# DavidHuji/CapDec

Measured on AMD Instinct MI355X. Metric: captions/sec (whole node), COCO-val 5k, prefix_len=10 beam=5, 1/2/4/8 GPUs, higher is better.
Workload: dtype f32 (operands split into 2 fp16 planes, 3 fp16 MFMAs per product, fp32 accumulate); 1 GPU; COCO-val-5k-shaped: 5000 x 512-d synthetic CLIP embeddings in total (sharded over the ranks) -> normalise -> TransformerMapper(8 layers) -> GPT-2 small KV-cached beam-5 decode, prefix_len 10, entry_length 67, hot-init seeded weights (never emit the stop id: all 67 steps run); captions_per_gpu=5000, beam=5, parallelism=caption-shard dp1

## Files before the change

capdec_amd/csrc/attention.hip:

```cpp
#include <cstdlib>

#include "bf16x3.h"
#include "common.h"

namespace capdec {

constexpr int ATT_CTX_MAX = 1024;
#define ATT_BIG_LDS(K, bytes)                                                                                   \
    if ((bytes) > 64 * 1024)                                                                                    \
    CAPDEC_HIP(hipFuncSetAttribute((const void *)(K), hipFuncAttributeMaxDynamicSharedMemorySize, (int)(bytes)))
constexpr int ATT_MFMA_MIN_P = 24;
constexpr int ATT_MFMA_MAX_P = 128;

__device__ __forceinline__ float dot4(const float4 &a, const float4 &b) {
    return (a.x * b.x + a.y * b.y) + (a.z * b.z + a.w * b.w);
}
__device__ __forceinline__ float group16_sum(float v) { return row16_sum(v); }
__device__ __forceinline__ float groups4_sum(float v) {
    v += __shfl_xor(v, 16, 64);
    v += __shfl_xor(v, 32, 64);
    return v;
}

template <typename KV> struct KvIo;
// ... 467 lines not shown
#pragma unroll
    for (int t = 0; t < NT; ++t) {
        if (t < nt) {
#pragma unroll
            for (int s2 = 0; s2 < 2; ++s2) {
                f16x8 ph, pl;
#pragma unroll
                for (int e = 0; e < 8; ++e) {
                    const float p = sc[t][8 * s2 + e];
                    if constexpr (SPLIT) {
                        const _Float16 hh = p < 0x1p-14f ? (_Float16)0.f : (_Float16)p;
                        ph[e] = hh;
                        pl[e] = (_Float16)((p - (float)hh) * H2_LO_SCALE);
                    } else
                        ph[e] = (_Float16)p;
                }
#pragma unroll
                for (int n = 0; n < 2; ++n) {
                    const _Float16 *vr = Vt + (size_t)(32 * n + l32) * VST + 32 * t + 16 * s2 + 8 * half;
                    const f16x8 vh = *reinterpret_cast<const f16x8 *>(vr);
                    if constexpr (SPLIT) {
                        const f16x8 vl = *reinterpret_cast<const f16x8 *>(vr + (size_t)64 * VST);
                        oc[n] = __builtin_amdgcn_mfma_f32_32x32x16_f16(pl, vh, oc[n], 0, 0, 0);
                        om[n] = __builtin_amdgcn_mfma_f32_32x32x16_f16(ph, vh, om[n], 0, 0, 0);
                        oc[n] = __builtin_amdgcn_mfma_f32_32x32x16_f16(ph, vl, oc[n], 0, 0, 0);
                    } else
                        om[n] = __builtin_amdgcn_mfma_f32_32x32x16_f16(ph, vh, om[n], 0, 0, 0);
                }
            }
        }
    }
    __syncthreads();
    float *ost = reinterpret_cast<float *>(am_smem) + (size_t)wave * 32 * AM_OST;
#pragma unroll
    for (int r = 0; r < 16; ++r) {
        const int row = (r & 3) + 8 * (r >> 2) + 4 * half;
        const float li = __shfl(linv, row, 64);
#pragma unroll
        for (int n = 0; n < 2; ++n) ost[row * AM_OST + 32 * n + l32] = (SPLIT ? om[n][r] + oc[n][r] * LO : om[n][r]) * li;
    }
    __builtin_amdgcn_fence(__ATOMIC_RELEASE, "wavefront");
    __builtin_amdgcn_wave_barrier();
    __builtin_amdgcn_fence(__ATOMIC_ACQUIRE, "wavefront");
    for (int q = lane; q < 32 * 16; q += 64) {
        const int row = q >> 4, c4 = q & 15, grow = wave * 32 + row;
        if (grow >= S) continue;
        const float4 o = *reinterpret_cast<const float4 *>(ost + row * AM_OST + c4 * 4);
        const int orow = cap * S + grow;
        if (packed_out) x3_store_quad(packed_out, d >> 4, orow, head * 4 + (c4 >> 2), c4 & 3, o, fmt);
        else reinterpret_cast<float4 *>(out + (size_t)orow * d + head * 64)[c4] = o;
    }
}

template <typename KV>
__global__ void kv_scatter_prefill_kernel(const float *__restrict__ qkv, KV *__restrict__ kc,
                                          KV *__restrict__ vc, int ncap, int P, int beam, int heads, int ctx,
                                          int d) {
    const int nv = d / 4;
    const int i = blockIdx.x * blockDim.x + threadIdx.x;
    if (i >= ncap * P * nv) return;
    const int c4 = i % nv, row = i / nv;
    const int cap = row / P, pos = row - cap * P;
    const int head = (c4 * 4) / 64, within = (c4 * 4) % 64;
    const size_t o = (((size_t)cap * beam * heads + head) * ctx + pos) * 64 + within;
    const float *r = qkv + (size_t)row * 3 * d;
    KvIo<KV>::st4(kc + o, reinterpret_cast<const float4 *>(r + d)[c4]);
    KvIo<KV>::st4(vc + o, reinterpret_cast<const float4 *>(r + 2 * d)[c4]);
}

int launch_kv_scatter_prefill(hipStream_t st, const float *qkv, const KvCache &c, int layer, int ncap, int P,
                              int beam) {
    const int d = c.heads * c.hd;
    const int tot = ncap * P * (d / 4);
    if (tot <= 0) return 0;
    if (c.bf16)
        hipLaunchKernelGGL(kv_scatter_prefill_kernel<__bf16>, dim3((tot + 255) / 256), dim3(256), 0, st, qkv,
                           c.kp<__bf16>(layer), c.vp<__bf16>(layer), ncap, P, beam, c.heads, c.ctx, d);
    else
        hipLaunchKernelGGL(kv_scatter_prefill_kernel<float>, dim3((tot + 255) / 256), dim3(256), 0, st, qkv,
                           c.kp<float>(layer), c.vp<float>(layer), ncap, P, beam, c.heads, c.ctx, d);
    CAPDEC_HIP(hipGetLastError());
    return 0;
}

int launch_attn_prefill(hipStream_t st, const float *qkv, const KvCache &c, int layer, int ncap, int P, int beam,
                        float *out, bool causal, void *packed_out, int fmt) {
    CAPDEC_CHECK(c.hd == 64, "attention: head_dim must be 64");
    CAPDEC_CHECK(P <= ATT_CTX_MAX && P <= c.ctx, "attention: prefix longer than the supported context");
    (void)layer; (void)beam;
    const bool tower = c.k == nullptr;
    const bool split = !((fmt == PK_F16X1 || fmt == PK_BF16X1) && tower);
    if (!c.bf16 && (P >= ATT_MFMA_MIN_P || tower) && P <= ATT_MFMA_MAX_P && ncap > 0) {
        const int nqt = (P + 31) / 32;
        const size_t lds = attn_mfma_lds_bytes(P, split ? 2 : 1);
#define LAUNCH_AM(CZ, NTV)                                                                                          \
    {                                                                                                               \
        if (lds > 64 * 1024)       \
            CAPDEC_HIP(hipFuncSetAttribute((const void *)attn_prefill_mfma_kernel<CZ, NTV, true>,                   \
                                           hipFuncAttributeMaxDynamicSharedMemorySize, (int)lds));                  \
        if (split)                                                                                                  \
            hipLaunchKernelGGL((attn_prefill_mfma_kernel<CZ, NTV, true>), dim3(ncap * c.heads), dim3(64 * nqt), lds, st, qkv, \
                               c.heads, P, c.heads * c.hd, out, (char *)packed_out, fmt);                            \
        else                                                                                                        \
            hipLaunchKernelGGL((attn_prefill_mfma_kernel<CZ, NTV, false>), dim3(ncap * c.heads), dim3(64 * nqt), lds, st, qkv, \
                               c.heads, P, c.heads * c.hd, out, (char *)packed_out, fmt);                            \
    }
#define LAUNCH_AM_NT(CZ)                                                                                            \
    switch (nqt) {                                                                                                  \
        case 1: LAUNCH_AM(CZ, 1) break;                                                                             \
        case 2: LAUNCH_AM(CZ, 2) break;                                                                             \
        case 3: LAUNCH_AM(CZ, 3) break;                                                                             \
        default: LAUNCH_AM(CZ, 4) break;                                                                            \
    }
        if (causal) { LAUNCH_AM_NT(true) } else { LAUNCH_AM_NT(false) }
#undef LAUNCH_AM_NT
#undef LAUNCH_AM
        CAPDEC_HIP(hipGetLastError());
        return 0;
    }
    constexpr int R = 8;
    const int total = ncap * c.heads * ((P + R - 1) / R);
    if (total <= 0) return 0;
    const size_t lds = (size_t)4 * R * P * sizeof(float);
    CAPDEC_CHECK(lds <= 160 * 1024, "attention: prefix too long for the score rows in LDS");
    ATT_BIG_LDS((attn_prefill_rows_kernel<R, __bf16>), lds);
    ATT_BIG_LDS((attn_prefill_rows_kernel<R, float>), lds);
    if (c.bf16)
        hipLaunchKernelGGL((attn_prefill_rows_kernel<R, __bf16>), dim3((total + 3) / 4), dim3(256), lds, st, qkv, total,
                           c.heads, P, c.heads * c.hd, causal ? 1 : 0, out, (char *)packed_out, fmt);
    else
        hipLaunchKernelGGL((attn_prefill_rows_kernel<R, float>), dim3((total + 3) / 4), dim3(256), lds, st, qkv, total,
                           c.heads, P, c.heads * c.hd, causal ? 1 : 0, out, (char *)packed_out, fmt);
    CAPDEC_HIP(hipGetLastError());
    return 0;
}

template <typename KV>
static int attn_decode_typed(hipStream_t st, const float *qkv, const KvCache &c, int layer, int rows, int beam, int L,
                             const uint8_t *anc, int anc_stride, float *out, void *packed_out, const int *cmap,
                             int fmt, bool cur_cached) {
    KV *kl = c.kp<KV>(layer), *vl = c.vp<KV>(layer);
    const int npre = anc == nullptr ? L : c.prefix_len;
    {
        const int ncap = rows / beam, total = ncap * c.heads;
        if (total <= 0) return 0;
        size_t lds = ((size_t)4 * beam * L * sizeof(int) + 1023) & ~(size_t)1023;
        CAPDEC_CHECK(lds + 32 * 1024 <= 160 * 1024, "attention: context too long for the slot table in LDS");
        dim3 grid((total + 3) / 4), block(256);
        const bool na4 = !c.fixed_variant && total <= 16384;
#define LAUNCH_BEAMS_V(B, OCC, NAV, CURV)                                                                       \
    ATT_BIG_LDS((attn_decode_beams_kernel<B, KV, OCC, NAV, CURV, false>), lds);                                    \
    hipLaunchKernelGGL((attn_decode_beams_kernel<B, KV, OCC, NAV, CURV, false>), grid, block, lds, st, qkv, kl, vl, total, \
                       c.heads, c.ctx, c.heads * c.hd, L, anc, anc_stride, out, (char *)packed_out, cmap, fmt, npre, 0)
#define LAUNCH_BEAMS_DMA(B, OCC)                                                                                \
    ATT_BIG_LDS((attn_decode_beams_kernel<B, float, OCC, 2, true, true>), lds + 4 * 2 * (2 * 2 * 1024));          \
    hipLaunchKernelGGL((attn_decode_beams_kernel<B, float, OCC, 2, true, true>), grid, block, lds + 4 * 2 * (2 * 2 * 1024), st, \
                       qkv, (float *)kl, (float *)vl, total, c.heads, c.ctx, c.heads * c.hd, L, anc, anc_stride, out,  \
                       (char *)packed_out, cmap, fmt, npre, (int)lds)
#define LAUNCH_BEAMS_NA(B, OCC, CURV)                                                                           \
    if constexpr (B <= 5) {                                                                                     \
        if (na4) { LAUNCH_BEAMS_V(B, OCC, 4, CURV); } else { LAUNCH_BEAMS_V(B, OCC, 2, CURV); }                 \
    } else { LAUNCH_BEAMS_V(B, OCC, 2, CURV); }
#define LAUNCH_BEAMS(B, OCC)                                                                                    \
    if constexpr (B == 1 || B == 5) {                                                                           \
        if (!cur_cached) { LAUNCH_BEAMS_NA(B, OCC, false) }                                                     \
        else if constexpr (sizeof(KV) == 4) { LAUNCH_BEAMS_DMA(B, OCC); }                                       \
        else { LAUNCH_BEAMS_NA(B, OCC, true) }                                                                  \
    } else { LAUNCH_BEAMS_NA(B, OCC, false) }
        switch (beam) {
            case 1: LAUNCH_BEAMS(1, 4); break;
            case 2: LAUNCH_BEAMS(2, 4); break;
// ... 25 lines not shown
}

__global__ __launch_bounds__(256) void attn_mapper_kernel(const float *__restrict__ q, int ldq,
                                                          const float *__restrict__ k, const float *__restrict__ v,
                                                          int ldkv, float *__restrict__ out, int seq, int heads,
                                                          int hd, float scale) {
    extern __shared__ __attribute__((aligned(16))) float sm[];
    const int ld = hd + 1;
    float *Ks = sm;
    float *Vs = Ks + seq * ld;
    float *qb = Vs + seq * ld;
    float *pb = qb + 4 * hd;
    const int cap = blockIdx.x / heads, head = blockIdx.x - cap * heads;
    const int d = heads * hd;
    const int lane = threadIdx.x & 63, wave = threadIdx.x >> 6;
    for (int i = threadIdx.x; i < seq * hd; i += 256) {
        const int j = i / hd, c = i - j * hd;
        const size_t o = ((size_t)cap * seq + j) * ldkv + head * hd + c;
        Ks[j * ld + c] = k[o];
        Vs[j * ld + c] = v[o];
    }
    __syncthreads();
    for (int i = wave; i < seq; i += 4) {
        const float *qr = q + ((size_t)cap * seq + i) * ldq + head * hd;
        for (int c = lane; c < hd; c += 64) qb[wave * hd + c] = qr[c];
        __builtin_amdgcn_wave_barrier();
        float mx = -INFINITY;
        for (int j = lane; j < seq; j += 64) {
            float s = 0.f;
            for (int c = 0; c < hd; ++c) s += qb[wave * hd + c] * Ks[j * ld + c];
            s *= scale;
            pb[wave * seq + j] = s;
            mx = fmaxf(mx, s);
        }
        mx = wave_max(mx);
        float sum = 0.f;
        for (int j = lane; j < seq; j += 64) {
            const float e = expf(pb[wave * seq + j] - mx);
            pb[wave * seq + j] = e;
            sum += e;
        }
        sum = wave_sum(sum);
        __builtin_amdgcn_wave_barrier();
        const float inv = 1.0f / sum;
        for (int c = lane; c < hd; c += 64) {
            float a = 0.f;
            for (int j = 0; j < seq; ++j) a += pb[wave * seq + j] * Vs[j * ld + c];
            out[((size_t)cap * seq + i) * d + head * hd + c] = a * inv;
        }
        __builtin_amdgcn_wave_barrier();
    }
}

int launch_attn_mapper(hipStream_t st, const float *q, int ldq, const float *k, const float *v, int ldkv, float *out,
                       int n, int seq, int heads, int hd) {
    if (n <= 0) return 0;
    const size_t lds = ((size_t)2 * seq * (hd + 1) + 4 * hd + 4 * seq) * sizeof(float);
    CAPDEC_CHECK(lds <= 160 * 1024, "mapper attention: sequence too long for LDS");
    if (lds > 64 * 1024)
        CAPDEC_HIP(hipFuncSetAttribute((const void *)attn_mapper_kernel, hipFuncAttributeMaxDynamicSharedMemorySize,
                                       (int)lds));
    hipLaunchKernelGGL(attn_mapper_kernel, dim3(n * heads), dim3(256), lds, st, q, ldq, k, v, ldkv, out, seq, heads, hd,
                       (float)pow((double)hd, -0.5));
    CAPDEC_HIP(hipGetLastError());
    return 0;
}

__global__ __launch_bounds__(256) void attn_cross_kernel(const float *__restrict__ q, int ldq, size_t q_cap,
                                                         const float *__restrict__ k, const float *__restrict__ v,
                                                         int ldkv, float *__restrict__ out, int total, int nq, int nkv,
                                                         int heads, int hd, float scale, int group, int tj, int vec) {
    extern __shared__ __attribute__((aligned(16))) float sm[];
    const int ld = hd + 1;
    const int tpu = 256 / group, wpu = tpu >> 6;
    const int ul = threadIdx.x / tpu, tu = threadIdx.x - ul * tpu;
    const int unit = blockIdx.x * group + ul;
    const bool live = unit < total;
    float *Ks = sm + (size_t)ul * (2 * nkv * ld + nq * hd + wpu * nkv);
    float *Vs = Ks + nkv * ld;
    float *Qs = Vs + nkv * ld;
    const int cap = unit / heads, head = unit - cap * heads;
    const int lane = tu & 63, wave = tu >> 6;
    float *pw = Qs + nq * hd + wave * nkv;
    if (live) {
        const float *kb = k + (size_t)cap * nkv * ldkv + head * hd, *vb = v + (size_t)cap * nkv * ldkv + head * hd;
        const float *qb = q + (size_t)cap * q_cap + head * hd;
        if (vec) {
            const int hv = hd >> 2;
            for (int i = tu; i < nkv * hv; i += tpu) {
                const int j = i / hv, c = (i - j * hv) << 2;
                const float4 a = *reinterpret_cast<const float4 *>(kb + (size_t)j * ldkv + c);
                const float4 b = *reinterpret_cast<const float4 *>(vb + (size_t)j * ldkv + c);
                float *kd = Ks + j * ld + c, *vd = Vs + j * ld + c;
                kd[0] = a.x; kd[1] = a.y; kd[2] = a.z; kd[3] = a.w;
                vd[0] = b.x; vd[1] = b.y; vd[2] = b.z; vd[3] = b.w;
            }
            for (int i = tu; i < nq * hv; i += tpu) {
                const int r = i / hv, c = (i - r * hv) << 2;
                const float4 a = *reinterpret_cast<const float4 *>(qb + (size_t)r * ldq + c);
                float *qd = Qs + r * hd + c;
                qd[0] = a.x; qd[1] = a.y; qd[2] = a.z; qd[3] = a.w;
            }
        } else {
            for (int i = tu; i < nkv * hd; i += tpu) {
                const int j = i / hd, c = i - j * hd;
                Ks[j * ld + c] = kb[(size_t)j * ldkv + c];
                Vs[j * ld + c] = vb[(size_t)j * ldkv + c];
            }
            for (int i = tu; i < nq * hd; i += tpu) {
// ... 79 lines not shown
```

capdec_amd/csrc/common.h:

```cpp
#pragma once
#include <hip/hip_runtime.h>
#include <stdint.h>
#include <string>
#include <type_traits>
#include <vector>

#include "../../include/capdec.h"
#include "config.h"

namespace capdec {

void set_error(const std::string &msg);

#define CAPDEC_HIP(expr)                                                                         \
    do {                                                                                         \
        hipError_t _e = (expr);                                                                  \
        if (_e != hipSuccess) {                                                                  \
            ::capdec::set_error(std::string(#expr) + ": " + hipGetErrorString(_e) + " (" +       \
                                __FILE__ + ":" + std::to_string(__LINE__) + ")");               \
            return 1;                                                                            \
        }                                                                                        \
    } while (0)

#define CAPDEC_CHECK(cond, msg)                                                                  \
// ... 158 lines not shown
                     int ldy, int rows, int d);
int launch_l2norm_rows(hipStream_t st, const float *x, void *packed, float *y, int rows, int d, int fmt, int *row_bad,
                       int *any_bad);
int launch_embed_tokens(hipStream_t st, const int *tok, const float *wte, const float *wpe_row, float *h, int rows,
                        int d, const int *cmap = nullptr, int beam = 1);
int launch_embed_prefix(hipStream_t st, const float *prefix, const float *wpe, float *h, int n, int P, int pos0,
                        int d);
int launch_gather_rows(hipStream_t st, const float *table, const int *ids, float *out, int rows, int d);
int launch_normalize_prefix(hipStream_t st, const float *x, int n, int dim, int normalize, const float *offset,
                            float *out);
int launch_noise_inject(hipStream_t st, const float *x, int n, int dim, float variance, const float *offset,
                        int uniform, int dont_norm, uint64_t seed, const float *noise, const float *u, float *out);
int launch_tmapper_concat(hipStream_t st, const float *lin, const float *prefix_const, float *seq, int n,
                          int clip_len, int P, int d);
int launch_tmapper_take(hipStream_t st, const float *seq, float *out, int n, int clip_len, int P, int d);
int launch_transpose(hipStream_t st, const float *in, float *out, int rows, int cols);
int launch_clip_text_embed(hipStream_t st, const int *tokens, const float *tok_emb, const float *pos_emb, float *h,
                           int n, int L, int d, int P = 0, const int *perm = nullptr);
int launch_eot_index(hipStream_t st, const int *tokens, int *flat_idx, int n, int L, int flat = 1);
int launch_eot_rows(hipStream_t st, const int *pos, const int *perm, int *rows, int m, int P);
int launch_scatter_rows(hipStream_t st, const float *src, const int *perm, float *dst, int rows, int d);
int launch_im2col_patches(hipStream_t st, const float *pixels, float *patches, int n, int S, int patch);
int launch_vision_assemble(hipStream_t st, const float *patch_out, const float *cls, const float *pos, float *seq,
                           int n, int ntok, int d);

int launch_conv3x3_packed(hipStream_t st, const void *act_pk, const void *Bpacked, float *C, int ldc, int Nimg, int H,
                          int W, int Cin, int Cout, const GemmEpilogue &epi, int fmt, const void *zeros, size_t zero_bytes);

int launch_im2col3x3(hipStream_t st, const float *in, float *out, int N, int H, int W, int C, int stride, bool nchw3,
                     int Kp);
int launch_im2col3x3_packed(hipStream_t st, const float *in, void *out, int N, int H, int W, int C, int stride, bool nchw3,
                            int Kp, int fmt);
int launch_avgpool2(hipStream_t st, const float *in, float *out, int N, int H, int W, int C);
int launch_avgpool2_packed(hipStream_t st, const void *in, void *out, int N, int H, int W, int C, int fmt);
int launch_unpack_rows(hipStream_t st, const void *in, float *out, int M, int C, int fmt);
int launch_attnpool_tokens(hipStream_t st, const float *feat, const float *pos, float *t, int N, int HW, int C);
int launch_attnpool_attend(hipStream_t st, const float *q, const float *k, const float *v, float *out, int N, int heads,
                           int T, int C);

struct KvCache {
    void *k = nullptr;
    void *v = nullptr;
    int rows = 0, heads = 0, ctx = 0, hd = 0;
    bool bf16 = false;
    int prefix_len = 0;
    bool fixed_variant = false;
    size_t layer_stride() const { return (size_t)rows * heads * ctx * hd; }
    size_t elem_bytes() const { return bf16 ? 2 : 4; }
    template <typename T> T *kp(int layer) const { return reinterpret_cast<T *>(k) + (size_t)layer * layer_stride(); }
    template <typename T> T *vp(int layer) const { return reinterpret_cast<T *>(v) + (size_t)layer * layer_stride(); }
};
int launch_kv_scatter_prefill(hipStream_t st, const float *qkv, const KvCache &c, int layer, int ncap, int P,
                              int beam);
int launch_attn_prefill(hipStream_t st, const float *qkv, const KvCache &c, int layer, int ncap, int P, int beam,
                        float *out, bool causal = true, void *packed_out = nullptr, int fmt = 0);
int launch_attn_decode(hipStream_t st, const float *qkv, const KvCache &c, int layer, int rows, int beam, int L,
                       const uint8_t *anc, int anc_stride, float *out, void *packed_out = nullptr,
                       const int *cmap = nullptr, int fmt = 0, bool cur_cached = false);
int launch_attn_mapper(hipStream_t st, const float *q, int ldq, const float *k, const float *v, int ldkv, float *out,
                       int n, int seq, int heads, int hd);
constexpr size_t ATTN_CROSS_GROUP_LDS = 26 * 1024;
size_t attn_cross_lds_bytes(int nq, int nkv, int hd, int group);
int launch_attn_cross(hipStream_t st, const float *q, int ldq, size_t q_cap_stride, const float *k, const float *v,
                      int ldkv, float *out, int n, int nq, int nkv, int heads, int hd);

int launch_topk_merge(hipStream_t st, const float *tile_max, const float *tile_sum, const float *cand_val,
                      const int *cand_idx, int rows, int ntiles, int k, float *lse, float *top_val, int *top_idx);
int launch_topk_merge_k3(hipStream_t st, const float *tile_max, const float *tile_sum, const float *cand_val,
                         const int *cand_idx, int rows, int ntiles, float *lse, float *top_val, int *top_idx,
                         int *flag_rows, int *flag_count, int *flag_total);
int launch_topk_merge_rows(hipStream_t st, const float *cand_val, const int *cand_idx, const int *count_dev,
                           const int *out_rows, int rows_cap, int ntiles, float *top_val, int *top_idx);
int launch_gather_packed_rows(hipStream_t st, const void *packed, int K, const int *src_rows, const int *count_dev,
                              int rows_cap, void *out, int fmt);
struct BeamState {
    int *tokens = nullptr;
    float *scores = nullptr;
    float *seq = nullptr;
    uint8_t *stopped = nullptr;
    uint8_t *done = nullptr;
    uint8_t *anc = nullptr;
    int *next_tok = nullptr;
    int *alive_count = nullptr;
    unsigned *kv_stat = nullptr;
    int diverge = 0;
    float *logp = nullptr;
};
int launch_beam_init(hipStream_t st, const BeamState &s, const float *lse, const float *top_val, const int *top_idx,
                     int ncap, int beam, int k, int T, int ctx, int P, int stop_id);
int launch_beam_step(hipStream_t st, const BeamState &s, const float *lse, const float *top_val, const int *top_idx,
                     int ncap, int beam, int k, int T, int ctx, int step, int pos_new, int vocab, int stop_id,
                     const int *cmap = nullptr);
int launch_beam_finalize(hipStream_t st, const BeamState &s, int ncap, int beam, int T, int *ids, int *lens,
                         float *scores, int *order);
int launch_group_beam_init(hipStream_t st, const BeamState &s, const float *lse, const float *top_val, const int *top_idx,
                           int ncap, int beam, int groups, float diversity, int k, int T, int ctx, int P, int stop_id);
int launch_group_beam_step(hipStream_t st, const BeamState &s, const float *lse, const float *top_val, const int *top_idx,
                           int ncap, int beam, int groups, float diversity, int k, int T, int ctx, int step, int pos_new,
                           int vocab, int stop_id, const int *cmap = nullptr);
int launch_group_beam_logp(hipStream_t st, const BeamState &s, int ncap, int beam, const int *order, float *logp_out);
struct GreedyState {
    int *ids = nullptr;
    int *lens = nullptr;
    uint8_t *done = nullptr;
    int *next_tok = nullptr;
    int *alive_count = nullptr;
    float *logp = nullptr;
    int T = 0, stop_id = -1, alt_stop_id = -1;
    const int *cmap = nullptr;
};
__device__ __forceinline__ void greedy_emit(const GreedyState &s, int row, int step, int tok, float lp) {
    s.next_tok[row] = tok;
    s.ids[(size_t)row * s.T + step] = tok;
// ... 46 lines not shown
```

capdec_amd/csrc/context.h:

```cpp
#pragma once
#include <rccl/rccl.h>

#include <algorithm>
#include <cmath>
#include <cstring>
#include <map>
#include <memory>
#include <utility>

#include "bf16x3.h"
#include "common.h"
#include "config.h"

namespace capdec {

struct DBuf {
    void *p = nullptr;
    size_t cap = 0;
    int ensure(size_t bytes) {
        if (bytes <= cap) return 0;
        if (p) CAPDEC_HIP(hipFree(p));
        p = nullptr;
        cap = 0;
        CAPDEC_HIP(hipMalloc(&p, bytes));
// ... 167 lines not shown
        (void)hipEventRecord(r.a, c->stream);
        c->prof.recs.push_back(r);
        idx = (int)c->prof.recs.size() - 1;
    }
    ~ProfScope() {
        if (idx >= 0) (void)hipEventRecord(c->prof.recs[idx].b, c->stream);
    }
};
int prof_collect(capdec_ctx *c);

void train_release(capdec_ctx *c);

void comm_release(capdec_ctx *c);

inline int pad64(int c) { return (c + 63) / 64 * 64; }

int upload(std::vector<void *> &owned, const float *h_src, size_t n, float **out);
int upload_transposed(capdec_ctx *c, std::vector<void *> &owned, const float *h_src, int rows, int cols, float **out);
void free_all(std::vector<void *> &owned);

void drop_planes(capdec_ctx *c);
void drop_planes_of(capdec_ctx *c, const void *weight);
int pack_fmt(const capdec_ctx *c);
inline bool mode_single(const capdec_ctx *c) { return c->gemm_mode == GEMM_BF16 || c->gemm_mode == GEMM_F16; }
int pack_any(capdec_ctx *c, const float *W, int N, int K, int fmt, void *out);
int planes_of(capdec_ctx *c, const float *W, int N, int K, bool cache, const void **out, int fmt_override = -1,
              bool *wide_ok = nullptr);
int gemm_family(int fmt);
int gemm_epilogue(capdec_ctx *c, GemmEpilogue &e, int M, int N, int K, bool split, bool invariant);
int gemm_native(capdec_ctx *c, const float *A, int lda, const float *Bt, int ldb, float *C, int ldc, int M, int N, int K,
                GemmEpilogue e = GemmEpilogue());
int gemm(capdec_ctx *c, const float *A, int lda, const float *Bt, int ldb, float *C, int ldc, int M, int N, int K,
         const float *bias, int act, const float *resid = nullptr, int ldr = 0, bool weight = true);
int gemm_tn(capdec_ctx *c, const float *Xa, int lda, const float *Xb, int ldb, int rows, int N1, int N2, float *C, int ldc);
bool use_packed_a(capdec_ctx *c, int K);
struct NextLn { const float *w, *b; float eps; int *done; };
int gemm_packed(capdec_ctx *c, const void *Apk, const float *W, float *C, int ldc, int M, int N, int K, const float *bias,
                int act, const float *resid = nullptr, int ldr = 0, void *packed_out = nullptr,
                const NextLn *next_ln = nullptr, const void *resid_packed = nullptr,
                const QkvScatter *qkv_scatter = nullptr);
int ln_gemm_packed(capdec_ctx *c, const float *h, int ldh, const float *lnw, const float *lnb, float eps, const float *W,
                   float *C, int ldc, int M, int N, int K, const float *bias, int act, void *packed_out = nullptr,
                   bool ln_ready = false, const QkvScatter *qkv_scatter = nullptr);

int topk_workspace(capdec_ctx *c, int rows, int ntiles, int k, TopkOut *o);
int ln_gemm_topk(capdec_ctx *c, const float *h, int ldh, const float *lnw, const float *lnb, float eps, const float *W,
                 int M, int N, int K, int k, float inv_temp, const TopkOut &o, bool k3_ok, bool *k3);
int gemm_topk_dev(capdec_ctx *c, const void *Apk, const float *W, const int *m_dev, int N, int K, float inv_temp,
                  const TopkOut &o);
bool topk_packed_a(const capdec_ctx *c, int K);
int gemm_topk(capdec_ctx *c, const void *A, const float *Bt, bool cache, bool b_small, int M, int N, int K, int k,
              const TopkOut &o, float *lse, float *top_val, int *top_idx);

struct TLayerBufs { const float *x; float *a1, *qkv; const float *att; float *mid, *a2, *ff, *out; };
int tlayer_self_front(capdec_ctx *c, const TMapLayer &w, const TLayerBufs &b, int M, int wd, bool weight);
int tlayer_tail(capdec_ctx *c, const TMapLayer &w, const TLayerBufs &b, int M, int wd, int hid, bool weight);

struct StepShape {
    bool prefill;
    int ncap, P, beam;
    int rows, L;
    const uint8_t *anc;
    int anc_stride;
    const int *cmap;
};
struct StackCfg {
    const std::vector<Gpt2Layer> *layers;
    int n_layer, d;
    float eps;
    int act;
    bool causal, keep_kv;
};
int ensure_body_ws(capdec_ctx *c, int M, int d);
int stack_body(capdec_ctx *c, const StackCfg &g, const StepShape &s, const KvCache &kv);
void kv_geometry(KvCache &kv, int rows, int ctx, int heads, int hd);
int gpt2_body(capdec_ctx *c, const StepShape &s, const KvCache &kv);
int lm_head_select(capdec_ctx *c, const float *h0, int ldh, int R, int k, float inv_temp);
int ensure_kv(capdec_ctx *c, KvCache &kv, int rows, int ctx, int heads = 0, int hd = 0, int layers = 0);

void drop_wte_norm(capdec_ctx *c);

}
```

capdec_amd/csrc/decode.hip:

```cpp
#include "context.h"

namespace capdec {

int ensure_body_ws(capdec_ctx *c, int M, int d) {
    CAPDEC_TRY(c->h.ensure((size_t)M * d * 4));
    CAPDEC_TRY(c->x.ensure((size_t)M * d * 4));
    CAPDEC_TRY(c->qkv.ensure((size_t)M * 3 * d * 4));
    CAPDEC_TRY(c->att.ensure((size_t)M * d * 4));
    CAPDEC_TRY(c->ff.ensure((size_t)M * 4 * d * 4));
    return 0;
}

int stack_body(capdec_ctx *c, const StackCfg &g, const StepShape &s, const KvCache &kv) {
    const int d = g.d, M = s.prefill ? s.ncap * s.P : s.rows;
    float *h = c->h.as<float>(), *x = c->x.as<float>(), *qkv = c->qkv.as<float>(), *att = c->att.as<float>(),
          *ff = c->ff.as<float>();
    const bool chain = use_packed_a(c, d) && c->pack_chain;
    const bool kv_direct = c->tune.kv_direct;
    void *apk = nullptr, *fpk = nullptr;
    if (chain) {
        CAPDEC_TRY(c->apk.ensure(x3_packed_bytes_host(M, d)));
        CAPDEC_TRY(c->fpk.ensure(x3_packed_bytes_host(M, 4 * d)));
        apk = c->apk.p;
        fpk = c->fpk.p;
    }
    int ln1_ready = 0;
    for (int l = 0; l < g.n_layer; ++l) {
        const Gpt2Layer &w = (*g.layers)[l];
        const int kl = g.keep_kv ? l : 0;
        QkvScatter sc;
        const bool mode_ok = (c->gemm_mode == GEMM_F16X2 && !kv.bf16) || (c->gemm_mode == GEMM_BF16 && kv.bf16);
        const bool scatter = kv_direct && !s.prefill && g.keep_kv && mode_ok && use_packed_a(c, d) && w.bqkv &&
                             (((uintptr_t)w.bqkv | (uintptr_t)qkv) & 15) == 0 &&
                             d % GEMM_BN == 0 && (s.beam == 1 || s.beam == 5) &&
                             (c->batch_invariant || gemm_splitk_slices(M, 3 * d, d, c->tune) == 1);
        if (scatter) {
            sc.kc = reinterpret_cast<float *>(kv.bf16 ? (void *)kv.kp<__bf16>(kl) : (void *)kv.kp<float>(kl));
            sc.vc = reinterpret_cast<float *>(kv.bf16 ? (void *)kv.vp<__bf16>(kl) : (void *)kv.vp<float>(kl));
            sc.cmap = s.cmap;
            sc.beam = s.beam; sc.heads = kv.heads; sc.ctx = kv.ctx; sc.pos = s.L - 1; sc.d = d;
            sc.bf16 = kv.bf16;
        }
        if (use_packed_a(c, d)) {
            CAPDEC_TRY(ln_gemm_packed(c, h, d, w.ln1w, w.ln1b, g.eps, w.wqkv, qkv, 3 * d, M, 3 * d, d, w.bqkv, CAPDEC_ACT_NONE,
                                      nullptr, ln1_ready != 0, scatter ? &sc : nullptr));
            ln1_ready = 0;
        } else {
            { ProfScope ps(c, F_LN); CAPDEC_TRY(launch_layernorm(c->stream, h, d, w.ln1w, w.ln1b, g.eps, x, d, M, d)); }
            CAPDEC_TRY(gemm(c, x, d, w.wqkv, d, qkv, 3 * d, M, 3 * d, d, w.bqkv, CAPDEC_ACT_NONE));
        }
        if (s.prefill) {
            ProfScope ps(c, F_ATTN_PRE);
            if (g.keep_kv)
                CAPDEC_TRY(launch_kv_scatter_prefill(c->stream, qkv, kv, kl, s.ncap, s.P, s.beam));
            CAPDEC_TRY(launch_attn_prefill(c->stream, qkv, kv, kl, s.ncap, s.P, s.beam, att, g.causal, apk, pack_fmt(c)));
        } else {
            ProfScope ps(c, F_ATTN_DEC);
            CAPDEC_TRY(launch_attn_decode(c->stream, qkv, kv, kl, s.rows, s.beam, s.L, s.anc, s.anc_stride, att, apk, s.cmap, pack_fmt(c),
                                          scatter));
        }
        int ln2_ready = 0;
        if (chain) {
            const NextLn n2{w.ln2w, w.ln2b, g.eps, &ln2_ready};
            CAPDEC_TRY(gemm_packed(c, apk, w.wproj, h, d, M, d, d, w.bproj, CAPDEC_ACT_NONE, h, d, nullptr, &n2));
        } else {
            CAPDEC_TRY(gemm(c, att, d, w.wproj, d, h, d, M, d, d, w.bproj, CAPDEC_ACT_NONE, h, d));
        }
        if (chain) {
            CAPDEC_TRY(ln_gemm_packed(c, h, d, w.ln2w, w.ln2b, g.eps, w.wfc, ff, 4 * d, M, 4 * d, d, w.bfc, g.act, fpk,
                                      ln2_ready != 0));
            const bool has_next = l + 1 < g.n_layer;
            const NextLn n1{has_next ? (*g.layers)[l + 1].ln1w : nullptr, has_next ? (*g.layers)[l + 1].ln1b : nullptr, g.eps,
                            &ln1_ready};
            CAPDEC_TRY(gemm_packed(c, fpk, w.wproj2, h, d, M, d, 4 * d, w.bproj2, CAPDEC_ACT_NONE, h, d, nullptr,
                                   has_next ? &n1 : nullptr));
            continue;
        }
        if (use_packed_a(c, d)) {
            CAPDEC_TRY(ln_gemm_packed(c, h, d, w.ln2w, w.ln2b, g.eps, w.wfc, ff, 4 * d, M, 4 * d, d, w.bfc, g.act));
        } else {
            { ProfScope ps(c, F_LN); CAPDEC_TRY(launch_layernorm(c->stream, h, d, w.ln2w, w.ln2b, g.eps, x, d, M, d)); }
            CAPDEC_TRY(gemm(c, x, d, w.wfc, d, ff, 4 * d, M, 4 * d, d, w.bfc, g.act));
        }
        CAPDEC_TRY(gemm(c, ff, 4 * d, w.wproj2, 4 * d, h, d, M, d, 4 * d, w.bproj2, CAPDEC_ACT_NONE, h, d));
    }
    return 0;
}

int gpt2_body(capdec_ctx *c, const StepShape &s, const KvCache &kv) {
    const Gpt2 &g = c->gpt;
    StackCfg cfg{&g.layers, g.n_layer, g.d, g.eps, CAPDEC_ACT_GELU_NEW, true, true};
    return stack_body(c, cfg, s, kv);
}

int lm_head_select(capdec_ctx *c, const float *h0, int ldh, int R, int k, float inv_temp) {
    const Gpt2 &g = c->gpt;
    const int d = g.d, nt = gemm_tiles_n(g.vocab);
    TopkOut o;
    CAPDEC_TRY(topk_workspace(c, R, nt, k, &o));
    CAPDEC_TRY(c->topv.ensure((size_t)R * k * 4));
    CAPDEC_TRY(c->topi.ensure((size_t)R * k * 4));
    bool k3 = false;
    CAPDEC_TRY(ln_gemm_topk(c, h0, ldh, g.lnfw, g.lnfb, g.eps, g.wte, R, g.vocab, d, k, inv_temp, o,
                            c->tune.lmhead_k3 && k == 5 && !c->k3_off, &k3));
    if (k3) {
        CAPDEC_TRY(c->lmflag.ensure(((size_t)R + 2) * 4));
// ... 455 lines not shown
```

capdec_amd/csrc/mapper.hip:

```cpp
#include "context.h"

namespace capdec {

int tlayer_self_front(capdec_ctx *c, const TMapLayer &w, const TLayerBufs &b, int M, int wd, bool weight) {
    CAPDEC_CHECK(w.fused, "mapper: a layer without the fused [q | k | v] projection has no self front");
    { ProfScope ps(c, F_LN); CAPDEC_TRY(launch_layernorm(c->stream, b.x, wd, w.n1w, w.n1b, 1e-5f, b.a1, wd, M, wd)); }
    return gemm(c, b.a1, wd, w.wq, wd, b.qkv, 3 * wd, M, 3 * wd, wd, nullptr, CAPDEC_ACT_NONE, nullptr, 0, weight);
}

int tlayer_tail(capdec_ctx *c, const TMapLayer &w, const TLayerBufs &b, int M, int wd, int hid, bool weight) {
    CAPDEC_TRY(gemm(c, b.att, wd, w.wproj, wd, b.mid, wd, M, wd, wd, w.bproj, CAPDEC_ACT_NONE, b.x, wd, weight));
    { ProfScope ps(c, F_LN); CAPDEC_TRY(launch_layernorm(c->stream, b.mid, wd, w.n2w, w.n2b, 1e-5f, b.a2, wd, M, wd)); }
    CAPDEC_TRY(gemm(c, b.a2, wd, w.wfc1, wd, b.ff, hid, M, hid, wd, w.bfc1, CAPDEC_ACT_RELU, nullptr, 0, weight));
    return gemm(c, b.ff, hid, w.wfc2, hid, b.out, wd, M, wd, hid, w.bfc2, CAPDEC_ACT_NONE, b.mid, wd, weight);
}

static int encdec_chunk(capdec_ctx *c, const float *x, int n, float *out) {
    Mapper &m = c->map;
    const int d = m.d, E = m.enc_dim, C = m.clip_len, P = m.P, L = m.n_layers, H = m.heads;
    const int Me = n * C, Md = n * P;
    CAPDEC_CHECK(attn_cross_lds_bytes(C, C, E / H, 1) <= 160 * 1024 && attn_cross_lds_bytes(P, C, d / H, 1) <= 160 * 1024 &&
                 attn_cross_lds_bytes(P, P, d / H, 1) <= 160 * 1024, "mapper_forward: one head's keys, values and queries exceed 160 KB of LDS");
    const size_t ldc = (size_t)L * 2 * d;
    CAPDEC_TRY(c->m_lin.ensure((size_t)Me * E * 4));
    CAPDEC_TRY(c->m_seq.ensure((size_t)Md * d * 4));
    CAPDEC_TRY(c->m_x.ensure(std::max((size_t)Me * E, (size_t)Md * d) * 4));
    CAPDEC_TRY(c->m_qkv.ensure(std::max((size_t)Me * 3 * E, (size_t)Md * 3 * d) * 4));
    CAPDEC_TRY(c->m_att.ensure(std::max((size_t)Me * E, (size_t)Md * d) * 4));
    CAPDEC_TRY(c->m_ff.ensure(std::max((size_t)Me * m.enc_hidden, (size_t)Md * m.mlp_hidden) * 4));
    CAPDEC_TRY(c->m_kvc.ensure((size_t)Me * ldc * 4));
    CAPDEC_TRY(c->m_hid.ensure((size_t)2 * P * d * 4));
    float *ref = c->m_lin.as<float>(), *seq = c->m_seq.as<float>(), *xn = c->m_x.as<float>(), *qkv = c->m_qkv.as<float>(),
          *att = c->m_att.as<float>(), *ff = c->m_ff.as<float>(), *kvc = c->m_kvc.as<float>(), *q0 = c->m_hid.as<float>();
    CAPDEC_TRY(gemm(c, x, m.D, m.lin_w, m.D, ref, C * E, n, C * E, m.D, m.lin_b, CAPDEC_ACT_NONE));
    const TLayerBufs eb{ref, xn, qkv, att, ref, xn, ff, ref};
    for (int l = 0; l < L; ++l) {
        CAPDEC_TRY(tlayer_self_front(c, m.layers[l], eb, Me, E, true));
        { ProfScope ps(c, F_MAP_ATTN); CAPDEC_TRY(launch_attn_cross(c->stream, qkv, 3 * E, (size_t)C * 3 * E, qkv + E, qkv + 2 * E, 3 * E, att, n, C, C, H, E / H)); }
        CAPDEC_TRY(tlayer_tail(c, m.layers[l], eb, Me, E, m.enc_hidden, true));
    }
    CAPDEC_TRY(gemm(c, ref, E, m.wkv_cross, E, kvc, (int)ldc, Me, (int)ldc, E, nullptr, CAPDEC_ACT_NONE));
    { ProfScope ps(c, F_OTHER); CAPDEC_TRY(launch_tmapper_concat(c->stream, nullptr, m.prefix_const, seq, n, 0, P, d)); }
    float *q = qkv, *kv = qkv + (size_t)Md * d;
    for (int l = 0; l < 2 * L; ++l) {
        const TMapLayer &w = m.dec[l];
        const bool cross = l % 2 == 0;
        const float *ql = q;
        size_t q_cap = (size_t)P * d;
        if (l == 0) {
            { ProfScope ps(c, F_LN); CAPDEC_TRY(launch_layernorm(c->stream, m.prefix_const, d, w.n1w, w.n1b, 1e-5f, q0 + (size_t)P * d, d, P, d)); }
            CAPDEC_TRY(gemm(c, q0 + (size_t)P * d, d, w.wq, d, q0, d, P, d, d, nullptr, CAPDEC_ACT_NONE));
            ql = q0;
            q_cap = 0;
        } else {
            { ProfScope ps(c, F_LN); CAPDEC_TRY(launch_layernorm(c->stream, seq, d, w.n1w, w.n1b, 1e-5f, xn, d, Md, d)); }
            CAPDEC_TRY(gemm(c, xn, d, w.wq, d, q, d, Md, d, d, nullptr, CAPDEC_ACT_NONE));
        }
        if (cross) {
            const float *kl = kvc + (size_t)(l / 2) * 2 * d;
            { ProfScope ps(c, F_MAP_ATTN); CAPDEC_TRY(launch_attn_cross(c->stream, ql, d, q_cap, kl, kl + d, (int)ldc, att, n, P, C, H, d / H)); }
        } else {
            CAPDEC_TRY(gemm(c, seq, d, w.wkv, d, kv, 2 * d, Md, 2 * d, d, nullptr, CAPDEC_ACT_NONE));
            { ProfScope ps(c, F_MAP_ATTN); CAPDEC_TRY(launch_attn_cross(c->stream, ql, d, q_cap, kv, kv + d, 2 * d, att, n, P, P, H, d / H)); }
        }
        CAPDEC_TRY(tlayer_tail(c, w, TLayerBufs{seq, xn, nullptr, att, seq, xn, ff, l == 2 * L - 1 ? out : seq}, Md, d, m.mlp_hidden, true));
    }
    return 0;
}

static int mapper_chunk(capdec_ctx *c, const float *x, int n, float *out) {
    Mapper &m = c->map;
    const int d = m.d;
    if (m.kind == 3) return encdec_chunk(c, x, n, out);
    if (m.kind == 1) {
        CAPDEC_TRY(c->m_hid.ensure((size_t)n * m.hidden * 4));
        CAPDEC_TRY(gemm(c, x, m.D, m.w1, m.D, c->m_hid.as<float>(), m.hidden, n, m.hidden, m.D, m.b1, CAPDEC_ACT_TANH));
        CAPDEC_TRY(gemm(c, c->m_hid.as<float>(), m.hidden, m.w2, m.hidden, out, m.P * d, n, m.P * d, m.hidden, m.b2,
                        CAPDEC_ACT_NONE));
        return 0;
    }
    const int S = m.clip_len + m.P, M = n * S, hd = d / m.heads;
    CAPDEC_TRY(c->m_lin.ensure((size_t)n * m.clip_len * d * 4));
    CAPDEC_TRY(c->m_seq.ensure((size_t)M * d * 4));
    CAPDEC_TRY(c->m_x.ensure((size_t)M * d * 4));
    CAPDEC_TRY(c->m_qkv.ensure((size_t)M * 3 * d * 4));
    CAPDEC_TRY(c->m_att.ensure((size_t)M * d * 4));
    CAPDEC_TRY(c->m_ff.ensure((size_t)M * m.mlp_hidden * 4));
    float *seq = c->m_seq.as<float>(), *xn = c->m_x.as<float>(), *qkv = c->m_qkv.as<float>(), *att = c->m_att.as<float>();
    CAPDEC_TRY(gemm(c, x, m.D, m.lin_w, m.D, c->m_lin.as<float>(), m.clip_len * d, n, m.clip_len * d, m.D, m.lin_b,
                    CAPDEC_ACT_NONE));
    { ProfScope ps(c, F_OTHER); CAPDEC_TRY(launch_tmapper_concat(c->stream, c->m_lin.as<float>(), m.prefix_const, seq, n, m.clip_len, m.P, d)); }
    const TLayerBufs b{seq, xn, qkv, att, seq, xn, c->m_ff.as<float>(), seq};
    for (int l = 0; l < m.n_layers; ++l) {
        CAPDEC_TRY(tlayer_self_front(c, m.layers[l], b, M, d, true));
        { ProfScope ps(c, F_MAP_ATTN); CAPDEC_TRY(launch_attn_mapper(c->stream, qkv, 3 * d, qkv + d, qkv + 2 * d, 3 * d, att, n, S, m.heads, hd)); }
        CAPDEC_TRY(tlayer_tail(c, m.layers[l], b, M, d, m.mlp_hidden, true));
    }
    { ProfScope ps(c, F_OTHER); CAPDEC_TRY(launch_tmapper_take(c->stream, seq, out, n, m.clip_len, m.P, d)); }
    return 0;
}

}

using namespace capdec;

extern "C" {

int capdec_normalize_prefix(capdec_ctx *c, const float *x, int n, int dim, int normalize, const float *offset,
                            float *out) {
    CAPDEC_CHECK(c && n >= 0 && dim >= 1 && (n == 0 || (x && out)), "normalize_prefix: bad argument");
    if (n == 0) return 0;
    CAPDEC_HIP(hipSetDevice(c->device));
    ProfScope ps(c, F_OTHER);
    return launch_normalize_prefix(c->stream, x, n, dim, normalize, offset, out);
}

int capdec_noise_inject(capdec_ctx *c, const float *x, int n, int dim, float variance, const float *offset,
                        int uniform, int dont_norm, uint64_t seed, const float *noise, const float *u, float *out) {
    CAPDEC_CHECK(c && n >= 0 && dim >= 1 && (n == 0 || (x && out)), "noise_inject: bad argument");
    CAPDEC_CHECK(variance >= 0.f, "noise_inject: negative variance");
    if (n == 0) return 0;
    CAPDEC_HIP(hipSetDevice(c->device));
    ProfScope ps(c, F_OTHER);
    return launch_noise_inject(c->stream, x, n, dim, variance, offset, uniform, dont_norm, seed, noise, u, out);
}

int capdec_mapper_forward(capdec_ctx *c, const float *x, int n, float *out) {
    CAPDEC_CHECK(c && c->map.kind != 0, "mapper_forward: no mapper loaded");
    CAPDEC_CHECK(n >= 0 && (n == 0 || (x && out)), "mapper_forward: bad argument");
    CAPDEC_HIP(hipSetDevice(c->device));
    const Mapper &m = c->map;
    const int chunk = 8192;
    for (int c0 = 0; c0 < n; c0 += chunk) {
        const int nc = std::min(chunk, n - c0);
        CAPDEC_TRY(mapper_chunk(c, x + (size_t)c0 * m.D, nc, out + (size_t)c0 * m.P * m.d));
    }
    return 0;
}

}
```

Measured before the change: 3036 captions/s.

## Add lane-per-row attention kernel, fuse KV scatter into prefill, pack mapper layer chain

Adds a one-row-per-lane attention kernel that stages K/V in LDS. It is used for short GPT-2 prefixes, where it also writes the KV cache and so replaces the separate scatter launch, and for the 96-wide-head mapper attention. The mapper transformer layers now keep layernorm, attention and fc1 outputs in the packed f16x2 operand format and feed them straight into packed GEMMs, which avoids repacking fp32 activations before each GEMM. In exchange the code gains new dispatch paths and alignment and geometry conditions, and the scalar per-lane attention may be slower than the previous kernels at some shapes.

```diff
diff --git a/capdec_amd/csrc/attention.hip b/capdec_amd/csrc/attention.hip
--- a/capdec_amd/csrc/attention.hip
+++ b/capdec_amd/csrc/attention.hip
@@ -543,6 +543,138 @@
     }
 }
 
+template <int HD>
+__global__ __launch_bounds__(64) void attn_lane_rows_kernel(const float *__restrict__ q, int ldq,
+                                                            const float *__restrict__ k, const float *__restrict__ v,
+                                                            int ldkv, int total, int seq, int heads, int U, float qscale,
+                                                            int causal, float *__restrict__ out, char *__restrict__ packed_out,
+                                                            int fmt, float *__restrict__ kc, float *__restrict__ vc,
+                                                            int beam, int ctx) {
+    extern __shared__ __attribute__((aligned(16))) float lr_sm[];
+    constexpr int H4 = HD / 4;
+    const int ust = seq * HD + 4;
+    float *Ks = lr_sm, *Vs = Ks + (size_t)U * ust, *sc = Vs + (size_t)U * ust;
+    const int lane = threadIdx.x;
+    const int unit0 = blockIdx.x * U;
+    const int nu = min(U, total - unit0);
+    const int d = heads * HD;
+    const int nquad = nu * seq * H4;
+    int c4 = lane % H4, j, u, cap, head;
+    {
+        const int row = lane / H4;
+        u = row / seq; j = row - u * seq;
+        const int unit = unit0 + u;
+        cap = unit / heads; head = unit - cap * heads;
+    }
+    for (int i0 = 0; i0 < nquad; i0 += 64 * 4) {
+        float4 kk[4], vv[4];
+        int lo[4];
+        size_t co[4];
+#pragma unroll
+        for (int t = 0; t < 4; ++t) {
+            const bool in = i0 + t * 64 + lane < nquad;
+            const int ce = in ? c4 : H4 - 1, je = in ? j : seq - 1, ue = in ? u : nu - 1;
+            int cape = cap, heade = head;
+            if (!in) { const int unit = unit0 + nu - 1; cape = unit / heads; heade = unit - cape * heads; }
+            const size_t g = ((size_t)cape * seq + je) * ldkv + heade * HD + ce * 4;
+            kk[t] = *reinterpret_cast<const float4 *>(k + g);
+            vv[t] = *reinterpret_cast<const float4 *>(v + g);
+            lo[t] = ue * ust + je * HD + ce * 4;
+            co[t] = (((size_t)cape * beam * heads + heade) * ctx + je) * HD + ce * 4;
+            c4 += 64 % H4;
+            j += 64 / H4;
+            if (c4 >= H4) { c4 -= H4; ++j; }
+            while (j >= seq) {
+                j -= seq; ++u;
+                if (++head == heads) { head = 0; ++cap; }
+            }
+        }
+#pragma unroll
+        for (int t = 0; t < 4; ++t) {
+            if (i0 + t * 64 + lane < nquad) {
+                *reinterpret_cast<float4 *>(Ks + lo[t]) = kk[t];
+                *reinterpret_cast<float4 *>(Vs + lo[t]) = vv[t];
+                if (kc) {
+                    *reinterpret_cast<float4 *>(kc + co[t]) = kk[t];
+                    *reinterpret_cast<float4 *>(vc + co[t]) = vv[t];
+                }
+            }
+        }
+    }
+    __syncthreads();
+    for (int qc = 0; qc < seq; qc += 64) {
+        int u = 0, i = qc + lane;
+        if (seq <= 64) { u = lane / seq; i = lane - u * seq; }
+        const bool valid = u < nu && i < seq;
+        if (!valid) { u = 0; i = 0; }
+        const int unit = unit0 + u, cap = unit / heads, head = unit - cap * heads;
+        const size_t row = (size_t)cap * seq + i;
+        const float *qr = q + row * ldq + head * HD;
+        float4 qv[H4];
+#pragma unroll
+        for (int c = 0; c < H4; ++c) {
+            qv[c] = *reinterpret_cast<const float4 *>(qr + c * 4);
+            qv[c].x *= qscale; qv[c].y *= qscale; qv[c].z *= qscale; qv[c].w *= qscale;
+        }
+        const int Lk = causal ? i + 1 : seq;
+        const float *Ku = Ks + u * ust, *Vu = Vs + u * ust;
+        float mx = ATT_NEG;
+        for (int j = 0; j < seq; ++j) {
+            float4 a = make_float4(0.f, 0.f, 0.f, 0.f);
+#pragma unroll
+            for (int c = 0; c < H4; ++c) {
+                const float4 kv4 = *reinterpret_cast<const float4 *>(Ku + j * HD + c * 4);
+                a.x += qv[c].x * kv4.x; a.y += qv[c].y * kv4.y; a.z += qv[c].z * kv4.z; a.w += qv[c].w * kv4.w;
+            }
+            const float s = j < Lk ? (a.x + a.y) + (a.z + a.w) : ATT_NEG;
+            sc[j * 64 + lane] = s;
+            mx = fmaxf(mx, s);
+        }
+        float4 acc[H4];
+#pragma unroll
+        for (int c = 0; c < H4; ++c) acc[c] = make_float4(0.f, 0.f, 0.f, 0.f);
+        float sum = 0.f;
+        for (int j = 0; j < seq; ++j) {
+            const float s = sc[j * 64 + lane];
+            const float p = j < Lk ? att_exp2(s - mx) : 0.f;
+            sum += p;
+#pragma unroll
+            for (int c = 0; c < H4; ++c) {
+                const float4 vv4 = *reinterpret_cast<const float4 *>(Vu + j * HD + c * 4);
+                acc[c].x += p * vv4.x; acc[c].y += p * vv4.y; acc[c].z += p * vv4.z; acc[c].w += p * vv4.w;
+            }
+        }
+        if (valid) {
+            const float inv = 1.0f / sum;
+#pragma unroll
+            for (int c = 0; c < H4; ++c) {
+                const float4 o = make_float4(acc[c].x * inv, acc[c].y * inv, acc[c].z * inv, acc[c].w * inv);
+                const int col = head * HD + c * 4;
+                if (packed_out) x3_store_quad(packed_out, d >> 4, (int)row, col >> 4, (col >> 2) & 3, o, fmt);
+                else *reinterpret_cast<float4 *>(out + row * d + col) = o;
+            }
+        }
+    }
+}
+
+inline int attn_lane_units(int seq) { return seq >= 64 ? 1 : 64 / seq; }
+inline size_t attn_lane_lds_bytes(int seq, int hd) {
+    return ((size_t)2 * attn_lane_units(seq) * ((size_t)seq * hd + 4) + (size_t)seq * 64) * sizeof(float);
+}
+template <int HD>
+static int launch_attn_lane_rows(hipStream_t st, const float *q, int ldq, const float *k, const float *v, int ldkv, int n,
+                                 int seq, int heads, float scale, bool causal, float *out, void *packed_out, int fmt,
+                                 float *kc, float *vc, int beam, int ctx) {
+    const int U = attn_lane_units(seq), total = n * heads;
+    const size_t lds = attn_lane_lds_bytes(seq, HD);
+    ATT_BIG_LDS(attn_lane_rows_kernel<HD>, lds);
+    hipLaunchKernelGGL(attn_lane_rows_kernel<HD>, dim3((total + U - 1) / U), dim3(64), lds, st, q, ldq, k, v, ldkv, total,
+                       seq, heads, U, scale * 1.4426950408889634f, causal ? 1 : 0, out, (char *)packed_out, fmt, kc, vc, beam,
+                       ctx);
+    CAPDEC_HIP(hipGetLastError());
+    return 0;
+}
+
 template <typename KV>
 __global__ void kv_scatter_prefill_kernel(const float *__restrict__ qkv, KV *__restrict__ kc,
                                           KV *__restrict__ vc, int ncap, int P, int beam, int heads, int ctx,
@@ -574,11 +706,14 @@
     return 0;
 }
 
+bool attn_prefill_writes_kv(const KvCache &c, int P) {
+    return c.k != nullptr && !c.bf16 && c.hd == 64 && P >= 1 && P < ATT_MFMA_MIN_P;
+}
+
 int launch_attn_prefill(hipStream_t st, const float *qkv, const KvCache &c, int layer, int ncap, int P, int beam,
                         float *out, bool causal, void *packed_out, int fmt) {
     CAPDEC_CHECK(c.hd == 64, "attention: head_dim must be 64");
     CAPDEC_CHECK(P <= ATT_CTX_MAX && P <= c.ctx, "attention: prefix longer than the supported context");
-    (void)layer; (void)beam;
     const bool tower = c.k == nullptr;
     const bool split = !((fmt == PK_F16X1 || fmt == PK_BF16X1) && tower);
     if (!c.bf16 && (P >= ATT_MFMA_MIN_P || tower) && P <= ATT_MFMA_MAX_P && ncap > 0) {
@@ -608,6 +743,12 @@
 #undef LAUNCH_AM
         CAPDEC_HIP(hipGetLastError());
         return 0;
+    }
+    if (attn_prefill_writes_kv(c, P)) {
+        if (ncap <= 0) return 0;
+        const int d = c.heads * c.hd;
+        return launch_attn_lane_rows<64>(st, qkv, 3 * d, qkv + d, qkv + 2 * d, 3 * d, ncap, P, c.heads, 0.125f, causal, out,
+                                         packed_out, fmt, c.kp<float>(layer), c.vp<float>(layer), beam, c.ctx);
     }
     constexpr int R = 8;
     const int total = ncap * c.heads * ((P + R - 1) / R);
@@ -739,9 +880,16 @@
     }
 }
 
+bool attn_mapper_packs(int seq, int hd) { return hd == 96 && attn_lane_lds_bytes(seq, 96) <= 160 * 1024; }
+
 int launch_attn_mapper(hipStream_t st, const float *q, int ldq, const float *k, const float *v, int ldkv, float *out,
-                       int n, int seq, int heads, int hd) {
+                       int n, int seq, int heads, int hd, void *packed_out, int fmt) {
     if (n <= 0) return 0;
+    if (hd == 96 && ldq % 4 == 0 && ldkv % 4 == 0 && ((((uintptr_t)q | (uintptr_t)k | (uintptr_t)v | (uintptr_t)out)) & 15) == 0 &&
+        attn_lane_lds_bytes(seq, 96) <= 160 * 1024)
+        return launch_attn_lane_rows<96>(st, q, ldq, k, v, ldkv, n, seq, heads, (float)pow((double)hd, -0.5), false, out,
+                                         packed_out, fmt, nullptr, nullptr, 0, 0);
+    CAPDEC_CHECK(packed_out == nullptr, "mapper attention: no packed output at this geometry");
     const size_t lds = ((size_t)2 * seq * (hd + 1) + 4 * hd + 4 * seq) * sizeof(float);
     CAPDEC_CHECK(lds <= 160 * 1024, "mapper attention: sequence too long for LDS");
     if (lds > 64 * 1024)
diff --git a/capdec_amd/csrc/common.h b/capdec_amd/csrc/common.h
--- a/capdec_amd/csrc/common.h
+++ b/capdec_amd/csrc/common.h
@@ -234,13 +234,15 @@
 };
 int launch_kv_scatter_prefill(hipStream_t st, const float *qkv, const KvCache &c, int layer, int ncap, int P,
                               int beam);
+bool attn_prefill_writes_kv(const KvCache &c, int P);
 int launch_attn_prefill(hipStream_t st, const float *qkv, const KvCache &c, int layer, int ncap, int P, int beam,
                         float *out, bool causal = true, void *packed_out = nullptr, int fmt = 0);
 int launch_attn_decode(hipStream_t st, const float *qkv, const KvCache &c, int layer, int rows, int beam, int L,
                        const uint8_t *anc, int anc_stride, float *out, void *packed_out = nullptr,
                        const int *cmap = nullptr, int fmt = 0, bool cur_cached = false);
+bool attn_mapper_packs(int seq, int hd);
 int launch_attn_mapper(hipStream_t st, const float *q, int ldq, const float *k, const float *v, int ldkv, float *out,
-                       int n, int seq, int heads, int hd);
+                       int n, int seq, int heads, int hd, void *packed_out = nullptr, int fmt = 0);
 constexpr size_t ATTN_CROSS_GROUP_LDS = 26 * 1024;
 size_t attn_cross_lds_bytes(int nq, int nkv, int hd, int group);
 int launch_attn_cross(hipStream_t st, const float *q, int ldq, size_t q_cap_stride, const float *k, const float *v,
diff --git a/capdec_amd/csrc/context.h b/capdec_amd/csrc/context.h
--- a/capdec_amd/csrc/context.h
+++ b/capdec_amd/csrc/context.h
@@ -243,7 +243,11 @@
 int gemm_topk(capdec_ctx *c, const void *A, const float *Bt, bool cache, bool b_small, int M, int N, int K, int k,
               const TopkOut &o, float *lse, float *top_val, int *top_idx);
 
-struct TLayerBufs { const float *x; float *a1, *qkv; const float *att; float *mid, *a2, *ff, *out; };
+struct TLayerBufs {
+    const float *x; float *a1, *qkv; const float *att; float *mid, *a2, *ff, *out;
+    void *npk = nullptr, *apk = nullptr, *fpk = nullptr;
+};
+bool tlayer_packed_ok(const capdec_ctx *c, const TMapLayer &w, int wd, int hid);
 int tlayer_self_front(capdec_ctx *c, const TMapLayer &w, const TLayerBufs &b, int M, int wd, bool weight);
 int tlayer_tail(capdec_ctx *c, const TMapLayer &w, const TLayerBufs &b, int M, int wd, int hid, bool weight);
 
diff --git a/capdec_amd/csrc/decode.hip b/capdec_amd/csrc/decode.hip
--- a/capdec_amd/csrc/decode.hip
+++ b/capdec_amd/csrc/decode.hip
@@ -51,7 +51,7 @@
         }
         if (s.prefill) {
             ProfScope ps(c, F_ATTN_PRE);
-            if (g.keep_kv)
+            if (g.keep_kv && !attn_prefill_writes_kv(kv, s.P))
                 CAPDEC_TRY(launch_kv_scatter_prefill(c->stream, qkv, kv, kl, s.ncap, s.P, s.beam));
             CAPDEC_TRY(launch_attn_prefill(c->stream, qkv, kv, kl, s.ncap, s.P, s.beam, att, g.causal, apk, pack_fmt(c)));
         } else {
diff --git a/capdec_amd/csrc/mapper.hip b/capdec_amd/csrc/mapper.hip
--- a/capdec_amd/csrc/mapper.hip
+++ b/capdec_amd/csrc/mapper.hip
@@ -2,16 +2,35 @@
 
 namespace capdec {
 
+bool tlayer_packed_ok(const capdec_ctx *c, const TMapLayer &w, int wd, int hid) {
+    return c->gemm_mode == GEMM_F16X2 && c->pack_chain && wd % 64 == 0 && hid % 64 == 0 && ((uintptr_t)w.bfc1 & 15) == 0;
+}
+
 int tlayer_self_front(capdec_ctx *c, const TMapLayer &w, const TLayerBufs &b, int M, int wd, bool weight) {
     CAPDEC_CHECK(w.fused, "mapper: a layer without the fused [q | k | v] projection has no self front");
+    if (b.npk) {
+        CAPDEC_CHECK(weight && tlayer_packed_ok(c, w, wd, wd), "mapper: the packed layer form needs cached weights in the f16x2 mode");
+        { ProfScope ps(c, F_LN); CAPDEC_TRY(launch_layernorm_packed(c->stream, b.x, wd, w.n1w, w.n1b, 1e-5f, b.npk, M, wd, PK_F16X2)); }
+        return gemm_packed(c, b.npk, w.wq, b.qkv, 3 * wd, M, 3 * wd, wd, nullptr, CAPDEC_ACT_NONE);
+    }
     { ProfScope ps(c, F_LN); CAPDEC_TRY(launch_layernorm(c->stream, b.x, wd, w.n1w, w.n1b, 1e-5f, b.a1, wd, M, wd)); }
     return gemm(c, b.a1, wd, w.wq, wd, b.qkv, 3 * wd, M, 3 * wd, wd, nullptr, CAPDEC_ACT_NONE, nullptr, 0, weight);
 }
 
 int tlayer_tail(capdec_ctx *c, const TMapLayer &w, const TLayerBufs &b, int M, int wd, int hid, bool weight) {
-    CAPDEC_TRY(gemm(c, b.att, wd, w.wproj, wd, b.mid, wd, M, wd, wd, w.bproj, CAPDEC_ACT_NONE, b.x, wd, weight));
-    { ProfScope ps(c, F_LN); CAPDEC_TRY(launch_layernorm(c->stream, b.mid, wd, w.n2w, w.n2b, 1e-5f, b.a2, wd, M, wd)); }
-    CAPDEC_TRY(gemm(c, b.a2, wd, w.wfc1, wd, b.ff, hid, M, hid, wd, w.bfc1, CAPDEC_ACT_RELU, nullptr, 0, weight));
+    CAPDEC_CHECK(!(b.npk || b.apk || b.fpk) || (weight && tlayer_packed_ok(c, w, wd, hid)),
+                 "mapper: the packed layer form needs cached weights in the f16x2 mode");
+    if (b.apk) CAPDEC_TRY(gemm_packed(c, b.apk, w.wproj, b.mid, wd, M, wd, wd, w.bproj, CAPDEC_ACT_NONE, b.x, wd));
+    else CAPDEC_TRY(gemm(c, b.att, wd, w.wproj, wd, b.mid, wd, M, wd, wd, w.bproj, CAPDEC_ACT_NONE, b.x, wd, weight));
+    if (b.npk) {
+        { ProfScope ps(c, F_LN); CAPDEC_TRY(launch_layernorm_packed(c->stream, b.mid, wd, w.n2w, w.n2b, 1e-5f, b.npk, M, wd, PK_F16X2)); }
+        CAPDEC_TRY(gemm_packed(c, b.npk, w.wfc1, b.ff, hid, M, hid, wd, w.bfc1, CAPDEC_ACT_RELU, nullptr, 0, b.fpk));
+    } else {
+        CAPDEC_CHECK(!b.fpk, "mapper: a packed fc1 output needs the packed norm in front of it");
+        { ProfScope ps(c, F_LN); CAPDEC_TRY(launch_layernorm(c->stream, b.mid, wd, w.n2w, w.n2b, 1e-5f, b.a2, wd, M, wd)); }
+        CAPDEC_TRY(gemm(c, b.a2, wd, w.wfc1, wd, b.ff, hid, M, hid, wd, w.bfc1, CAPDEC_ACT_RELU, nullptr, 0, weight));
+    }
+    if (b.fpk) return gemm_packed(c, b.fpk, w.wfc2, b.out, wd, M, wd, hid, w.bfc2, CAPDEC_ACT_NONE, b.mid, wd);
     return gemm(c, b.ff, hid, w.wfc2, hid, b.out, wd, M, wd, hid, w.bfc2, CAPDEC_ACT_NONE, b.mid, wd, weight);
 }
 
@@ -90,10 +109,18 @@
     CAPDEC_TRY(gemm(c, x, m.D, m.lin_w, m.D, c->m_lin.as<float>(), m.clip_len * d, n, m.clip_len * d, m.D, m.lin_b,
                     CAPDEC_ACT_NONE));
     { ProfScope ps(c, F_OTHER); CAPDEC_TRY(launch_tmapper_concat(c->stream, c->m_lin.as<float>(), m.prefix_const, seq, n, m.clip_len, m.P, d)); }
-    const TLayerBufs b{seq, xn, qkv, att, seq, xn, c->m_ff.as<float>(), seq};
+    TLayerBufs b{seq, xn, qkv, att, seq, xn, c->m_ff.as<float>(), seq};
+    bool packed = m.n_layers > 0 && attn_mapper_packs(S, hd);
+    for (int l = 0; l < m.n_layers; ++l) packed = packed && tlayer_packed_ok(c, m.layers[l], d, m.mlp_hidden);
+    if (packed) {
+        CAPDEC_TRY(c->xpk.ensure(x3_packed_bytes_host(M, d)));
+        CAPDEC_TRY(c->apk.ensure(x3_packed_bytes_host(M, d)));
+        CAPDEC_TRY(c->fpk.ensure(x3_packed_bytes_host(M, m.mlp_hidden)));
+        b.npk = c->xpk.p; b.apk = c->apk.p; b.fpk = c->fpk.p;
+    }
     for (int l = 0; l < m.n_layers; ++l) {
         CAPDEC_TRY(tlayer_self_front(c, m.layers[l], b, M, d, true));
-        { ProfScope ps(c, F_MAP_ATTN); CAPDEC_TRY(launch_attn_mapper(c->stream, qkv, 3 * d, qkv + d, qkv + 2 * d, 3 * d, att, n, S, m.heads, hd)); }
+        { ProfScope ps(c, F_MAP_ATTN); CAPDEC_TRY(launch_attn_mapper(c->stream, qkv, 3 * d, qkv + d, qkv + 2 * d, 3 * d, att, n, S, m.heads, hd, b.apk, PK_F16X2)); }
         CAPDEC_TRY(tlayer_tail(c, m.layers[l], b, M, d, m.mlp_hidden, true));
     }
     { ProfScope ps(c, F_OTHER); CAPDEC_TRY(launch_tmapper_take(c->stream, seq, out, n, m.clip_len, m.P, d)); }
```

Result: no change. 3055 captions/s (median of 6 runs) (+0.6%).
